# wengroup/matten

Measured on AMD Instinct MI355X. Metric: edge_tensor_products_per_sec, higher is better.
Workload: dtype f32; 1 GPU; configs[2]: synthetic fcc-64 crystals (64 atoms, cutoff 5 A, 1152 edges each), paper hparams lmax=4, eval forward backbone+out_layer, one batch per step per GPU; last conv layer run for its live outputs only (258/842 radial-weight columns: the irreps its only reader takes) -- `value` counts 4 edge-TP per edge all the same, `value_full_layers` is the rate with the full last layer; nodes_per_gpu=64000, edges_per_gpu=1152000, conv_layers=4

## Files before the change

### include/matten_hip.h

```cpp
#ifndef MATTEN_HIP_H
#define MATTEN_HIP_H

#include <stddef.h>
#include <stdint.h>

#ifdef __cplusplus
extern "C" {
#endif

typedef void* matten_stream_t;

#define MATTEN_OK 0
#define MATTEN_EINVAL (-1)
#define MATTEN_ELAUNCH (-2)
#define MATTEN_ENOMEM (-3)

int matten_abi_version(void);

#define MATTEN_RADIAL_MAX_MID 3

size_t matten_csr_workspace_bytes(int64_t n_edges, int64_t n_nodes);
int matten_csr_counting_max_avg_degree(void);
int matten_csr_build(const int64_t* edge_index, int64_t n_edges, int64_t n_nodes, int32_t* perm,
                     int32_t* rowptr, int32_t* src_sorted, void* workspace, size_t workspace_bytes,
// ... 59 lines not shown
                               matten_stream_t stream);
int matten_radial_hidden_deep(const float* geom_sorted, int64_t n_edges, int n_basis, float r_start, float r_end,
                              const float* w0p, int nb_pad, const float* w_mid, int n_mid, int hidden, uint16_t* h2s,
                              const float* h_scale, matten_stream_t stream);
int matten_radial_hidden_multi_deep(const float* geom_sorted, int64_t n_edges, int n_basis, float r_start, float r_end,
                                    const float* const* w0p, int nb_pad, const float* const* w_mid, int n_mid, int hidden,
                                    uint16_t* const* h2s, const float* const* h_scale, int n_layers,
                                    matten_stream_t stream);
int matten_tp_fused(const float* x, int64_t d_in, const uint16_t* h2s, const float* w2p, int64_t w_pad,
                    const float* sh_sorted, int64_t sh_stride, const int32_t* rowptr, const int32_t* src_sorted,
                    int64_t n_nodes, const int32_t* group_entries, const int32_t* unit_map, int64_t n_entries,
                    int64_t units_per_tile, int64_t lds_floats_per_wave, int64_t d_mid, float avg_num_neighbors,
                    const float* num_neigh, const uint16_t* a_split, const float* a_scale_inv,
                    float* agg , matten_stream_t stream);

int matten_tp_max_cols(void);
int matten_tp_max_cols_l0(void);
int matten_tp_max_cols_l1(void);
int matten_tp_groups_hash(void);

int matten_species_linear(const float* x, int64_t d_in, const int32_t* order, const int32_t* seg, int64_t n_species,
                          const float* wp, int64_t w_stride, const int32_t* segs, int64_t n_segs, int64_t d_out,
                          const float* add, int64_t add_ld, int64_t n_rows, float* out, matten_stream_t stream);

int matten_species_linear_rows(const float* x, int64_t d_in, const int32_t* order, const int32_t* seg, int64_t n_species,
                               const float* wp, int64_t w_stride, const int32_t* segs, int64_t n_segs, int64_t d_out,
                               const float* add, int64_t add_ld, int64_t n_rows, float* out, matten_stream_t stream);

int matten_gate_bn(const float* x, int64_t d_in, const int32_t* meta, int64_t d_out, const float* act_cst,
                   const float* running_mean, const float* running_var, const float* bn_weight,
// ... 274 lines not shown
```

### matten_amd/_lib.py

```python
from __future__ import annotations

import ctypes
import os
from ctypes import c_float, c_int, c_int32, c_int64, c_size_t, c_void_p

_HERE = os.path.dirname(os.path.abspath(__file__))
LIB_PATH = os.path.join(_HERE, "libmatten_hip.so")

ABI_VERSION = 47

P = c_void_p
SIGNATURES = {
    "matten_abi_version": (c_int, []),
    "matten_csr_workspace_bytes": (c_size_t, [c_int64, c_int64]),
    "matten_group_workspace_bytes": (c_size_t, [c_int64, c_int64]),
    "matten_csr_counting_max_avg_degree": (c_int, []),
    "matten_csr_build": (c_int, [P, c_int64, c_int64, P, P, P, P, c_size_t, P, P]),
    "matten_csr_split_bound": (c_int64, [c_int64, c_int64, c_int64]),
    "matten_csr_split": (c_int, [P, c_int64, c_int64, c_int64, P, P, P, P, P]),
    "matten_group_by_key": (c_int, [P, c_int64, c_int64, P, P, P, c_size_t, P, P]),
    "matten_species_embed": (c_int, [P, c_int64, P, c_int64, c_int64, c_int64, P, P, c_int64, P, P, P, P, P, P]),
    "matten_edge_geom": (c_int, [P, P, P, P, c_int64, P, P, c_int64, c_int64, c_int, c_int, c_float, c_float, P, P, c_int, P, P, P, P, P]),
    "matten_radial_mlp": (c_int, [P, c_int64, c_int, c_float, c_float, P, c_int, P, P, c_int, c_int, c_float, P, c_int, P]),
    "matten_radial_mlp_deep": (c_int, [P, c_int64, c_int, c_float, c_float, P, c_int, P, c_int, P, c_int, c_int, c_float, P, c_int,
# ... 2 lines not shown
    "matten_tp_paths": (c_int, [P, c_int64, P, c_int64, P, c_int64, P, P, c_int64, P, P, c_int64, c_int64, c_int64, c_float, P, P, c_int,
                                P]),
    "matten_radial_hidden_multi": (c_int, [P, c_int64, c_int, c_float, c_float, P, c_int, P, c_int, P, P, c_int, P]),
    "matten_radial_hidden_multi_deep": (c_int, [P, c_int64, c_int, c_float, c_float, P, c_int, P, c_int, c_int, P, P, c_int, P]),
    "matten_agg_linear_max_mt": (c_int, []),
    "matten_agg_linear_block_chunks": (c_int, []),
    "matten_agg_linear_lds_bytes": (c_size_t, [c_int64, c_int64, c_int64]),
    "matten_agg_linear_max_lds_bytes": (c_size_t, []),
    "matten_agg_linear": (c_int, [P, c_int64, P, P, c_int64, P, c_int64, P, c_int64, P, c_int64, P, c_int64, c_int64,
                                  c_int64, P, P]),
    "matten_agg_linear_gate": (c_int, [P, c_int64, P, P, c_int64, P, c_int64, P, c_int64, P, c_int64, P, c_int64, c_int64,
                                       c_int64, P, P, P, P, c_int64, P, P]),
    "matten_agg_linear_gate_sets": (c_int, []),
    "matten_radial_hidden": (c_int, [P, c_int64, c_int, c_float, c_float, P, c_int, P, c_int, P, P, P]),
    "matten_radial_hidden_deep": (c_int, [P, c_int64, c_int, c_float, c_float, P, c_int, P, c_int, c_int, P, P, P]),
    "matten_tp_max_cols": (c_int, []),
    "matten_tp_max_cols_l0": (c_int, []),
    "matten_tp_max_cols_l1": (c_int, []),
    "matten_tp_groups_hash": (c_int, []),
    "matten_tp_fused": (c_int, [P, c_int64, P, P, c_int64, P, c_int64, P, P, c_int64, P, P, c_int64, c_int64, c_int64, c_int64, c_float, P, P, P, P, P]),
    "matten_species_linear": (c_int, [P, c_int64, P, P, c_int64, P, c_int64, P, c_int64, c_int64, P, c_int64, c_int64, P, P]),
    "matten_species_linear_rows": (c_int, [P, c_int64, P, P, c_int64, P, c_int64, P, c_int64, c_int64, P, c_int64, c_int64, P, P]),
    "matten_radial_mlp_bwd_small_slices": (c_int64, [c_int64]),
    "matten_radial_mlp_bwd_w2_ranges": (c_int64, [c_int64, c_int64]),
    "matten_radial_mlp_bwd_w2_ranges_deep": (c_int64, [c_int64, c_int64, c_int]),
    "matten_radial_mlp_bwd": (c_int, [P, c_int64, c_int, c_float, c_float, P, c_int, P, P, c_int, c_int, c_int, P, c_int64,
                                      c_int, P, P, P, c_float, c_float, c_float, P, P, P]),
    "matten_radial_mlp_bwd_deep": (c_int, [P, c_int64, c_int, c_float, c_float, P, c_int, P, c_int, P, c_int, c_int, c_int, P,
                                           c_int64, c_int, P, P, P, c_float, c_float, c_float, P, P, P]),
    "matten_radial_pack": (c_int, [P, P, P, c_int, c_int, c_int, c_int, c_float, c_float, c_float, P, P, P, P]),
# ... 128 lines not shown
```

### matten_amd/csrc/tp_fused.hip

```cpp
#include "tp_walk.h"

namespace {

using namespace matten_walk;

constexpr int KIND_MERGED = 256;
struct StoreAgg {
    template <class G>
    __device__ __forceinline__ void store(const Args& a, const GroupEntry& ge, const float* __restrict__ acc,
                                          float a_scale_inv, int node, int j, int u, bool valid) const {
        if (TPF_LAB_NO_STORE ? (valid && acc[0] == 12345.678f) : valid) {
            const float nn = a.avg_nn > 0.0f ? a.avg_nn : a.num_neigh[node];
            const float norm = nn > 0.0f ? a_scale_inv / sqrtf(nn) : 0.0f;
            float* orow = a.agg + (int64_t)node * a.d_mid;
            const bool merged = (ge.kind & KIND_MERGED) != 0;
            const GroupEntry& g2 = (&ge)[merged ? 1 : 0];
            const bool second = merged && u >= 2;
            const unsigned mask = merged ? (second ? g2.mask : (unsigned)g2.w_base) : ge.mask;
            const int uc = second ? u - 2 : u;
#pragma unroll
            for (int cc = 0; cc < G::NC; ++cc) {
                if ((mask >> cc) & 1u) {
                    const int d3 = 2 * G::L3[cc] + 1;
                    const int ks = second ? g2.t_off[cc] : ge.t_off[cc];
// ... 22 lines not shown
    const int cu_log2 = ge.cu_log2;
    const int cu = 1 << cu_log2;
    const int npw = 64 >> cu_log2;
    const int ch_log2 = npw >= 16 ? 0 : (4 - (6 - cu_log2));
    const int CH = 1 << ch_log2;
    const int T = npw >= 16 ? (npw >> 4) : 1;
    const int ncols = ge.mul * NC;
    const int MT = (ncols + 15) >> 4;
    const int ycol = MT * 16;
    const int stride = MT * 16 + 32 + 4;

    const int j = lane >> cu_log2;
    const int u = lane & (cu - 1);
    const int g = lane >> 4, c = lane & 15;
    const int xcol = ge.x_off + u * G::D1;
    constexpr int CAPC = cap_channels(L1, NC);
    constexpr int MTMAX = (CAPC * NC + 15) / 16;
    f16x8 ah[MTMAX], al[MTMAX];
    float a_scale_inv;
    {
        float av[MTMAX][8];
        float amax = 0.0f;
#pragma unroll
        for (int mt = 0; mt < MTMAX; ++mt) {
#pragma unroll
            for (int kk = 0; kk < 8; ++kk) {
                const int k = 16 * (kk >> 2) + 4 * g + (kk & 3);
                av[mt][kk] = (mt < MT) ? a.w2p[(int64_t)k * a.w_pad + ge.w_base + mt * 16 + c] : 0.0f;
                amax = fmaxf(amax, fabsf(av[mt][kk]));
            }
// ... 61 lines not shown
        __builtin_amdgcn_s_waitcnt(0xc07f);
        __builtin_amdgcn_wave_barrier();
        for (int so = 0; so < CH; ++so) {
            const int s = s0 + so;
            if (s >= maxdeg) break;
            float x[G::D1];
#pragma unroll
            for (int i = 0; i < G::D1; ++i) x[i] = xn[i];
            {
                const float* xp = a.x + (int64_t)src_nn * a.d_in + xcol;
#pragma unroll
                for (int i = 0; i < G::D1; ++i) xn[i] = xp[i];
                src_nn = a.src_sorted[min(beg + s + 2, e_last)];
            }
            if (s < deg) {
                const float* wp = tile + ((j << ch_log2) + so) * stride + u * NC;
                const float* yp = tile + ((j << ch_log2) + so) * stride + ycol + G::Y0;
                float y[G::NY], w[NC];
#pragma unroll
                for (int jj = 0; jj < G::NY; ++jj) y[jj] = yp[jj];
#pragma unroll
                for (int cc = 0; cc < NC; ++cc) w[cc] = wp[cc];
                G::apply(mask, x, y, w, acc);
            }
        }
        __builtin_amdgcn_wave_barrier();
    }
    StoreAgg{}.store<G>(a, ge, acc, a_scale_inv, node, j, u, valid);
}

#define MATTEN_RGS_ARGS a, ge, tile, stage, (um >> 8) & 0xffff, tile_id, r, reps, lane, StoreAgg{}
#define MATTEN_RGS(L1, GI, TT, TD, P) \
    do { \
        using HM = HotMask<L1, GI>; \
        if (HM::M0 && ge.mask == HM::M0) run_group_shared<L1, GI, TT, TD, P, HM::M0>(MATTEN_RGS_ARGS); \
        else if (HM::M1 && ge.mask == HM::M1) run_group_shared<L1, GI, TT, TD, P, HM::M1>(MATTEN_RGS_ARGS); \
        else run_group_shared<L1, GI, TT, TD, P, 0u>(MATTEN_RGS_ARGS); \
    } while (0)
#if defined(MATTEN_LAB) && defined(TPF_ONLY_VARIANT)
#ifndef TPF_ONLY_MASK
#define TPF_ONLY_MASK 0
#endif
#define MATTEN_RGS_ONLY(L1, GI, TT, TD, P) run_group_shared<L1, GI, TT, TD, P, (unsigned)(TPF_ONLY_MASK)>(MATTEN_RGS_ARGS)
#define MATTEN_GROUP_CASE_SHARED(L1, GI) \
    case (L1 * matten::GROUP_KIND_STRIDE + GI): \
        if (TPF_ONLY_VARIANT == 0) MATTEN_RGS_ONLY(L1, GI, 1, (TPF_CHUNK_DEEP && L1 == 0 ? 2 : 0), true); \
        else if (TPF_ONLY_VARIANT == 1) MATTEN_RGS_ONLY(L1, GI, 2, 0, false); \
        else if (TPF_ONLY_VARIANT == 2) MATTEN_RGS_ONLY(L1, GI, 1, (TPF_CHUNK_DEEP && L1 == 0 ? 2 : TwoDeepOk<L1, GI>::value ? 1 : 0), false); \
        else MATTEN_RGS_ONLY(L1, GI, 1, 0, false); \
        break;
#else
#define MATTEN_GROUP_CASE_SHARED(L1, GI) \
    case (L1 * matten::GROUP_KIND_STRIDE + GI): \
        if (paired && TPF_CHUNK_DEEP && L1 == 0 && nodes_per_wave <= 8 && nodes_per_wave >= 4) MATTEN_RGS(L1, GI, 1, (L1 == 0 ? 2 : 0), true); \
        else if (paired) MATTEN_RGS(L1, GI, 1, 0, true); \
        else if (nodes_per_wave > 16) MATTEN_RGS(L1, GI, 2, 0, false); \
        else if (TPF_CHUNK_DEEP && L1 == 0 && nodes_per_wave <= 8 && nodes_per_wave >= 4) MATTEN_RGS(L1, GI, 1, (L1 == 0 ? 2 : 0), false); \
        else if (TwoDeepOk<L1, GI>::value && nodes_per_wave <= 8 && nodes_per_wave >= TPF_TWO_DEEP_MIN_NPW) MATTEN_RGS(L1, GI, 1, (TwoDeepOk<L1, GI>::value ? 1 : 0), false); \
// ... 401 lines not shown
    if (grid >= ((int64_t)1 << 31)) return MATTEN_EINVAL;
#if TPF_TRACING
    a.trace = nullptr;
    if (g_tp_trace && grid * WAVES_PER_BLOCK <= g_tp_trace_waves) {
        if (g_tp_trace_skip <= 0) a.trace = g_tp_trace;
        if (g_tp_trace_skip == 0) g_tp_trace = nullptr;
        if (g_tp_trace_skip > 0) --g_tp_trace_skip;
    }
#endif
    tp_fused_kernel<<<(unsigned)grid, WAVES_PER_BLOCK * 64, lds, stream>>>(
        a, (const GroupEntry*)group_entries, unit_map, (int)n_entries, (int)units_per_tile, blocks_per_tile, n_tiles);
    MATTEN_LAUNCH_CHECK();
    return MATTEN_OK;
}

extern "C" int matten_tp_max_cols(void) { return TPF_MAX_COLS; }
extern "C" int matten_tp_max_cols_l0(void) { return TPF_MAX_COLS_L0; }
extern "C" int matten_tp_max_cols_l1(void) { return TPF_MAX_COLS_L1; }
extern "C" int matten_tp_groups_hash(void) { return matten::GROUPS_HASH; }
```

### matten_amd/csrc/tp_walk.h

```cpp
#pragma once
#include <type_traits>

#include "cg_gen.h"
#include "common.h"
#include "sh.h"

#ifndef MATTEN_LAB
#if defined(MATTEN_ABLATE_NO_GATHER) || defined(MATTEN_ABLATE_NO_XLOAD) || defined(MATTEN_ABLATE_NO_H2LOAD) || \
    defined(MATTEN_ABLATE_NO_MFMA) || defined(MATTEN_ABLATE_NO_VALU) || defined(MATTEN_ABLATE_NO_STORE) ||      \
    defined(MATTEN_ABLATE_NO_BARRIER) || defined(MATTEN_ABLATE_NO_LOOP) || defined(MATTEN_ABLATE_NO_EPI) || defined(MATTEN_ABLATE_ONE_YQUAD)
#error "MATTEN_ABLATE_* switches are honoured by -DMATTEN_LAB builds only (tools/*.sh)"
#endif
#endif
#if defined(MATTEN_LAB) && defined(MATTEN_ABLATE_NO_GATHER)
#define TPF_SRC(v) ((v) >= 0 ? (node < a.n_nodes ? node : 0) : 0)
#else
#define TPF_SRC(v) (v)
#endif
#if defined(MATTEN_LAB) && defined(MATTEN_ABLATE_NO_XLOAD)
#define TPF_XLD(xp, i, v) (1e-9f * (float)((v) + (i)))
#else
#define TPF_XLD(xp, i, v) ((xp)[i])
#endif
#if defined(MATTEN_LAB) && defined(MATTEN_ABLATE_NO_H2LOAD)
// ... 71 lines not shown

#ifndef TPF_SETPRIO
#define TPF_SETPRIO 3
#endif
#ifndef TPF_W_FIRST
#define TPF_W_FIRST 1
#endif
#ifndef TPF_W_FIRST2
#define TPF_W_FIRST2 1
#endif
#ifndef TPF_PAIR_SUM
#define TPF_PAIR_SUM 1
#endif
#ifndef TPF_EXACT_Y0
#define TPF_EXACT_Y0 0
#endif

#ifndef TPF_REP_PREFETCH
#define TPF_REP_PREFETCH 1
#endif
#ifndef TPF_MAX_COLS
#define TPF_MAX_COLS 64
#endif
#ifndef TPF_MAX_COLS_L0
#define TPF_MAX_COLS_L0 96
#endif
#ifndef TPF_MAX_COLS_L1
#define TPF_MAX_COLS_L1 TPF_MAX_COLS
#endif
__host__ __device__ constexpr int cap_channels(int l1, int nc) {
// ... 71 lines not shown
#pragma unroll
    for (int off = 32; off > 0; off >>= 1) maxdeg = max(maxdeg, __shfl_xor(maxdeg, off));
    if constexpr (TPF_LAB_NO_LOOP) maxdeg = 0;
    n.maxdeg = maxdeg;
    return n;
}
__device__ __forceinline__ UnitNodes unit_nodes(const Args& a, const GroupEntry& ge, int tile_id, int r, int lane) {
    return unit_nodes_finish(unit_nodes_issue(a, ge, tile_id, r, lane));
}

constexpr int STAGE_ROW = 68;
constexpr int STAGE_TMAX = 2;
constexpr int STAGE_FLOATS = 16 * STAGE_TMAX * STAGE_ROW;
constexpr int STAGE_TOTAL_FLOATS = 2 * STAGE_FLOATS;

template <int MTC>
__device__ __forceinline__ void mfma_tiles(const f16x8* __restrict__ ah, const f16x8* __restrict__ al, f16x8 bh, f16x8 bl,
                                           float* __restrict__ trow) {
    const f32x4 zero = {0.f, 0.f, 0.f, 0.f};
    f32x4 dx[MTC], dh[MTC];
#pragma unroll
    for (int mt = 0; mt < MTC; ++mt) {
        dx[mt] = __builtin_amdgcn_mfma_f32_16x16x32_f16(al[mt], bh, zero, 0, 0, 0);
        dh[mt] = __builtin_amdgcn_mfma_f32_16x16x32_f16(ah[mt], bh, zero, 0, 0, 0);
    }
#pragma unroll
    for (int mt = 0; mt < MTC; ++mt) dx[mt] = __builtin_amdgcn_mfma_f32_16x16x32_f16(ah[mt], bl, dx[mt], 0, 0, 0);
#pragma unroll
    for (int mt = 0; mt < MTC; ++mt) *reinterpret_cast<f32x4*>(trow + mt * 16) = dh[mt] + SPLIT_LO_INV * dx[mt];
}
// ... 6 lines not shown
    const char* safe;
    int64_t row_bytes;
    float* st_w;
    int beg_ld[TT], deg_ld[TT], so_ld[TT];
    int CH;
    f32x4 pf[TT];

    __device__ __forceinline__ void init(const Args& a, float* stage, int cu_log2, int beg, int deg_node) {
        const int npw = 64 >> cu_log2;
        const int ch_log2 = npw >= 16 ? 0 : 4 - (6 - cu_log2);
        CH = 1 << ch_log2;
        const int piece = threadIdx.x & 15;
        base = piece < 8 ? reinterpret_cast<const char*>(a.h2s) + piece * 16
                         : reinterpret_cast<const char*>(a.sh) + (piece - 8) * 16;
        row_bytes = piece < 8 ? (int64_t)(2 * HID * sizeof(_Float16)) : (int64_t)a.sh_stride * 4;
        safe = reinterpret_cast<const char*>(a.w2p);
        st_w = stage + (threadIdx.x >> 4) * STAGE_ROW + piece * 4;
#pragma unroll
        for (int t = 0; t < TT; ++t) {
            const int n = (int)(threadIdx.x >> 4) + 16 * t;
            const int jn = (n >> ch_log2) & (npw - 1);
            so_ld[t] = n & (CH - 1);
            beg_ld[t] = __shfl(beg, jn << cu_log2);
            deg_ld[t] = __shfl(deg_node, jn << cu_log2);
            pf[t] = f32x4{0.f, 0.f, 0.f, 0.f};
        }
    }
    __device__ __forceinline__ void issue(int s0) {
        if constexpr (TPF_LAB_NO_H2LOAD) return;
#pragma unroll
        for (int t = 0; t < TT; ++t)
// ... 22 lines not shown
        const int npw = 64 >> cu_log2;
        const int ch_log2 = 4 - (6 - cu_log2);
        CH = 1 << ch_log2;
        const int wave = threadIdx.x >> 6, lane = threadIdx.x & 63;
        if ((wave & 1) == 0 && (lane & ((1 << cu_log2) - 1)) == 0) {
            info[((wave >> 1) * 16 + (lane >> cu_log2)) * 2] = beg;
            info[((wave >> 1) * 16 + (lane >> cu_log2)) * 2 + 1] = deg_node;
            if (lane == 0) info[2 * 16 * 2 + (wave >> 1)] = my_maxdeg;
        }
        __syncthreads();
        maxdeg = max(info[2 * 16 * 2], info[2 * 16 * 2 + 1]);
        const int piece = threadIdx.x & 15;
        base = piece < 8 ? reinterpret_cast<const char*>(a.h2s) + piece * 16
                         : reinterpret_cast<const char*>(a.sh) + (piece - 8) * 16;
        row_bytes = piece < 8 ? (int64_t)(2 * HID * sizeof(_Float16)) : (int64_t)a.sh_stride * 4;
        safe = reinterpret_cast<const char*>(a.w2p);
        const int n = (int)(threadIdx.x >> 4);
        st_w = stage + n * STAGE_ROW + piece * 4;
        const int jn = (n >> ch_log2) & (npw - 1);
        so_ld = n & (CH - 1);
#pragma unroll
        for (int t = 0; t < 2; ++t) {
            beg_ld[t] = info[(t * 16 + jn) * 2];
            deg_ld[t] = info[(t * 16 + jn) * 2 + 1];
            pf[t] = f32x4{0.f, 0.f, 0.f, 0.f};
        }
    }
    __device__ __forceinline__ void issue(int s0) {
#pragma unroll
        for (int t = 0; t < 2; ++t)
            pf[t] = *reinterpret_cast<const f32x4*>(
// ... 36 lines not shown
        __syncthreads();
        int buf = 0;
        for (int s0 = 0; s0 < un.maxdeg; s0 += ld.CH, buf ^= 1) {
            ld.issue(s0 + ld.CH);
            ld.publish(buf ^ 1);
            __syncthreads();
        }
    }
}
__device__ __forceinline__ void run_loader_only(const Args& a, const GroupEntry& ge, float* __restrict__ stage, int tile_id,
                                                int r0, int reps, int lane) {
    if ((64 >> ge.cu_log2) > 16) run_loader_only_t<2>(a, ge, stage, tile_id, r0, reps, lane);
    else run_loader_only_t<1>(a, ge, stage, tile_id, r0, reps, lane);
}

template <int L1, int GI>
struct TwoDeepOk { static constexpr bool value = L1 == 0 || (L1 == 1 && (GI == 0 || TPF_PAIR_SUM)); };

template <int L1, int GI, int TT, int TWO_DEEP, bool PAIRED, unsigned CMASK, class Epilogue>
__device__ __forceinline__ void run_group_shared(const Args& a, const GroupEntry& ge, float* __restrict__ tile,
                                                 float* __restrict__ stage, int entry, int tile_id, int r0, int reps, int lane,
                                                 const Epilogue& epi) {
    static_assert(!PAIRED || TT == 1, "paired workgroups stage 2 x 16 rows");
#if TPF_TRACING
    const unsigned tr_in_hi = tpf_stamp_hi();
    const unsigned tr_in = tpf_stamp();
    unsigned tr_mfma = 0, tr_con = 0, tr_pub = 0, tr_bar = 0, tr_chunks = 0, tr_pro = 0, tr_epi = 0;
    unsigned tr_pro_pre = 0, tr_epi_sg = 0;
#endif
    const int row0 = PAIRED ? 16 * (int)(threadIdx.x >> 7) : 0;
    constexpr int STAGE_BUF = (PAIRED ? 32 : 16 * TT) * STAGE_ROW;
    using G = matten::Group<L1, GI>;
    constexpr int NC = G::NC;

    const unsigned mask = ge.mask;
    const int cu_log2 = ge.cu_log2;
    const int cu = 1 << cu_log2;
    const int npw = 64 >> cu_log2;
    const int ch_log2 = npw >= 16 ? 0 : 4 - (6 - cu_log2);
    const int CH = 1 << ch_log2;
    const int ncols = ge.mul * NC;
#if defined(MATTEN_LAB) && defined(TPF_ONLY_MT)
    const int MT = TPF_ONLY_MT;
#else
    const int MT = (ncols + 15) >> 4;
#endif

    const int j = lane >> cu_log2;
    const int u = lane & (cu - 1);
    const int g = lane >> 4, c = lane & 15;
    const int xcol = ge.x_off + u * G::D1;
    constexpr int CAPC = cap_channels(L1, NC);
    constexpr int MTMAX = (CAPC * NC + 15) / 16;
    const int stride = MT * 16 + 4;
    f16x8 ah[MTMAX], al[MTMAX];
    float a_scale_inv;
    if (a.a_split) {
        const f16x8* ap = reinterpret_cast<const f16x8*>(a.a_split) + ((int64_t)ge.a_tile * 64 + lane) * 2;
#pragma unroll
        for (int mt = 0; mt < MTMAX; ++mt) {
            const f16x8 z = {0, 0, 0, 0, 0, 0, 0, 0};
            ah[mt] = mt < MT ? ap[mt * 128] : z;
            al[mt] = mt < MT ? ap[mt * 128 + 1] : z;
        }
        a_scale_inv = a.a_scale_inv[entry];
    } else
    {
        float av[MTMAX][8];
        float amax = 0.0f;
// ... 12 lines not shown
        e = amax > 0.0f ? max(-100, min(100, e)) : 13;
        const float a_scale = __uint_as_float((unsigned)(127 + 13 - e) << 23);
        a_scale_inv = __uint_as_float((unsigned)(127 - 13 + e) << 23);
#pragma unroll
        for (int mt = 0; mt < MTMAX; ++mt) {
#pragma unroll
            for (int kk = 0; kk < 8; ++kk) {
                _Float16 hi, lo;
                split_f16(av[mt][kk] * a_scale, hi, lo);
                ah[mt][kk] = hi;
                al[mt][kk] = lo;
            }
        }
    }

    typename std::conditional<PAIRED, PairLoader, StageLoader<TT>>::type ld;
    static_assert(!TWO_DEEP || TwoDeepOk<L1, GI>::value, "two rows in flight only for the light kinds");
    static_assert(TWO_DEEP != 2 || G::D1 == 1, "a chunk of rows in flight: scalar input blocks");
    constexpr bool two_deep = TWO_DEEP == 1;
    constexpr bool chunk_deep = TWO_DEEP == 2;
    constexpr int XQ = 4;
    float xqa[XQ], xqb[XQ];
    int sq[XQ];
    int node, beg, deg, maxdeg, e_last;
    bool valid;
    float xn[G::D1], xb[G::D1];
    int src_nn, src_b = 0;
    auto start_group = [&](const UnitNodes& un) {
        node = un.node, beg = un.beg, valid = un.valid, maxdeg = un.maxdeg;
        deg = valid ? un.deg : 0;
// ... 51 lines not shown
#if TPF_TRACING
    const unsigned tr_loop = tpf_stamp();
    unsigned tr_a = tr_loop;
    tr_pro += (unsigned)(tr_loop - tr_rep);
#endif
    auto chunk_body = [&](const int s0, const int buf, float (&xcur)[XQ], float (&xnext)[XQ]) {
        __builtin_amdgcn_s_setprio(TPF_SETPRIO);
        ld.issue(s0 + CH);
        const float* sb = stage + buf * STAGE_BUF + row0 * STAGE_ROW;
#pragma unroll
        for (int t = 0; t < TT; ++t) {
            {
                const f16x8 bh = *reinterpret_cast<const f16x8*>(sb + (16 * t + c) * STAGE_ROW + g * 4);
                const f16x8 bl = *reinterpret_cast<const f16x8*>(sb + (16 * t + c) * STAGE_ROW + 16 + g * 4);
                if constexpr (TPF_LAB_NO_MFMA) {
                    if ((float)bh[0] == 12345.f) tile[c] = (float)bl[0];
                    continue;
                }
                float* trow = tile + (16 * t + c) * stride + 4 * g;
                if (MTMAX == 1 || MT == 1) mfma_tiles<1>(ah, al, bh, bl, trow);
                else if (MTMAX == 2 || MT == 2) mfma_tiles<(MTMAX < 2 ? MTMAX : 2)>(ah, al, bh, bl, trow);
                else if (MTMAX == 3 || MT == 3) mfma_tiles<(MTMAX < 3 ? MTMAX : 3)>(ah, al, bh, bl, trow);
                else if (MTMAX == 4 || MT == 4) mfma_tiles<(MTMAX < 4 ? MTMAX : 4)>(ah, al, bh, bl, trow);
                else if (MTMAX == 5 || MT == 5) mfma_tiles<(MTMAX < 5 ? MTMAX : 5)>(ah, al, bh, bl, trow);
                else if (MTMAX == 6 || MT == 6) mfma_tiles<(MTMAX < 6 ? MTMAX : 6)>(ah, al, bh, bl, trow);
                else mfma_tiles<MTMAX>(ah, al, bh, bl, trow);
            }
        }
        __builtin_amdgcn_s_waitcnt(0xc07f);
        __builtin_amdgcn_wave_barrier();
        __builtin_amdgcn_s_setprio(0);
#if TPF_TRACING
        const unsigned tr_b = tpf_stamp();
#endif
        auto contract = [&](int so, const float* __restrict__ x) {
            const float* wp = tile + ((j << ch_log2) + so) * stride + u * NC;
            const float* yp = sb + ((j << ch_log2) + so) * STAGE_ROW + 32 + G::Y0;
            float y[G::NY], w[NC];
            if constexpr (TPF_W_FIRST) {
#pragma unroll
                for (int cc = 0; cc < NC; ++cc) w[cc] = wp[cc];
                asm volatile("" ::: "memory");
            }
            if constexpr (TPF_EXACT_Y0 && L1 == 0 && G::Y0 == 0 && G::NY % 4 == 1) {
                y[G::NY - 1] = yp[G::NY - 1];
#pragma unroll
                for (int q = 0; q < G::NY / 4; ++q) {
                    const f32x4 v = reinterpret_cast<const f32x4*>(yp)[q];
                    y[4 * q] = v[0], y[4 * q + 1] = v[1], y[4 * q + 2] = v[2], y[4 * q + 3] = v[3];
                }
            } else
            {
                constexpr int Q0 = G::Y0 / 4 * 4, NQ = (G::Y0 + G::NY - Q0 + 3) / 4;
                float yq[4 * NQ];
                const f32x4* y4 = reinterpret_cast<const f32x4*>(yp - (G::Y0 - Q0));
#pragma unroll
                for (int q = 0; q < NQ; ++q) {
#if defined(MATTEN_LAB) && defined(MATTEN_ABLATE_ONE_YQUAD)
                    const f32x4 v0 = y4[0];
                    const f32x4 v = q == 0 ? v0 : v0 * (float)(q + 1);
#else
                    const f32x4 v = y4[q];
#endif
                    yq[4 * q] = v[0], yq[4 * q + 1] = v[1], yq[4 * q + 2] = v[2], yq[4 * q + 3] = v[3];
                }
#pragma unroll
                for (int jj = 0; jj < G::NY; ++jj) y[jj] = yq[G::Y0 - Q0 + jj];
            }
            if constexpr (!TPF_W_FIRST) {
#pragma unroll
                for (int cc = 0; cc < NC; ++cc) w[cc] = wp[cc];
            }
            G::apply(CMASK ? CMASK : mask, x, y, w, acc);
        };
        if constexpr (TPF_LAB_NO_VALU) {
        } else if constexpr (TWO_DEEP && TPF_PAIR_SUM && G::HAS_APPLY2) {
            auto fetch = [&](int so, float (&y)[G::NY], float (&w)[NC]) {
                const float* wp = tile + ((j << ch_log2) + so) * stride + u * NC;
                const float* yp = sb + ((j << ch_log2) + so) * STAGE_ROW + 32 + G::Y0;
                if constexpr (TPF_W_FIRST2) {
#pragma unroll
                    for (int cc = 0; cc < NC; ++cc) w[cc] = wp[cc];
                    asm volatile("" ::: "memory");
                }
                constexpr int Q0 = G::Y0 / 4 * 4, NQ = (G::Y0 + G::NY - Q0 + 3) / 4;
                float yq[4 * NQ];
                const f32x4* y4 = reinterpret_cast<const f32x4*>(yp - (G::Y0 - Q0));
#pragma unroll
                for (int q = 0; q < NQ; ++q) {
                    const f32x4 v = y4[q];
                    yq[4 * q] = v[0], yq[4 * q + 1] = v[1], yq[4 * q + 2] = v[2], yq[4 * q + 3] = v[3];
                }
#pragma unroll
                for (int jj = 0; jj < G::NY; ++jj) y[jj] = yq[G::Y0 - Q0 + jj];
                if constexpr (!TPF_W_FIRST2) {
#pragma unroll
                    for (int cc = 0; cc < NC; ++cc) w[cc] = wp[cc];
                }
            };
            for (int so = 0; so < CH; so += 2) {
                const int s = s0 + so;
                float ya[G::NY], wa[NC], yb[G::NY], wb[NC], xa[G::D1], xc[G::D1];
                fetch(so, ya, wa);
                fetch(so + 1, yb, wb);
#pragma unroll
                for (int i = 0; i < G::D1; ++i) xa[i] = s < deg ? xn[i] : 0.0f, xc[i] = s + 1 < deg ? xb[i] : 0.0f;
                {
                    const float* xp = a.x + (int64_t)TPF_SRC(src_nn) * a.d_in + xcol;
#pragma unroll
                    for (int i = 0; i < G::D1; ++i) xn[i] = TPF_XLD(xp, i, src_nn);
                    src_nn = a.src_sorted[min(beg + s + 4, e_last)];
                }
                {
                    const float* xp = a.x + (int64_t)TPF_SRC(src_b) * a.d_in + xcol;
#pragma unroll
                    for (int i = 0; i < G::D1; ++i) xb[i] = TPF_XLD(xp, i, src_b);
                    src_b = a.src_sorted[min(beg + s + 5, e_last)];
                }
                G::apply2(CMASK ? CMASK : mask, xa, ya, wa, xc, yb, wb, acc);
            }
        } else if constexpr (chunk_deep) {
#pragma unroll
            for (int i = 0; i < XQ; ++i) {
                const float* xp = a.x + (int64_t)TPF_SRC(sq[i]) * a.d_in + xcol;
                xnext[i] = TPF_XLD(xp, 0, sq[i]);
            }
#pragma unroll
            for (int i = 0; i < XQ; ++i) sq[i] = a.src_sorted[min(beg + s0 + 2 * CH + i, e_last)];
#pragma unroll
            for (int so = 0; so < XQ; ++so) {
                if (so < CH && s0 + so < deg) contract(so, xcur + so);
            }
        } else if (two_deep) {
            for (int so = 0; so < CH; so += 2) {
                const int s = s0 + so;
                if (s < deg) contract(so, xn);
                {
                    const float* xp = a.x + (int64_t)TPF_SRC(src_nn) * a.d_in + xcol;
#pragma unroll
                    for (int i = 0; i < G::D1; ++i) xn[i] = TPF_XLD(xp, i, src_nn);
                    src_nn = a.src_sorted[min(beg + s + 4, e_last)];
                }
                if (s + 1 < deg) contract(so + 1, xb);
                {
                    const float* xp = a.x + (int64_t)TPF_SRC(src_b) * a.d_in + xcol;
#pragma unroll
                    for (int i = 0; i < G::D1; ++i) xb[i] = TPF_XLD(xp, i, src_b);
                    src_b = a.src_sorted[min(beg + s + 5, e_last)];
                }
            }
        } else {
            for (int so = 0; so < CH; ++so) {
                const int s = s0 + so;
                if (s >= maxdeg) break;
                float x[G::D1];
#pragma unroll
                for (int i = 0; i < G::D1; ++i) x[i] = xn[i];
                {
                    const float* xp = a.x + (int64_t)TPF_SRC(src_nn) * a.d_in + xcol;
#pragma unroll
                    for (int i = 0; i < G::D1; ++i) xn[i] = TPF_XLD(xp, i, src_nn);
                    src_nn = a.src_sorted[min(beg + s + 2, e_last)];
                }
                if (s < deg) contract(so, x);
            }
// ... 94 lines not shown
```

### matten_amd/ops.py

```python
from __future__ import annotations

from typing import Optional, Tuple

import os

import numpy as np

import torch

from . import _lib
from .nn._tables import bump_weights_epoch


_EVENTS = None
_EVENTS_ONLY = None


def enable_event_timing(flag: bool = True, only=None) -> None:
    global _EVENTS, _EVENTS_ONLY
    _EVENTS = {} if flag else None
    _EVENTS_ONLY = tuple(only) if (flag and only) else None


def event_timings_ms():
# ... 540 lines not shown
_GROUPS_CHECKED = False


def tp_fused(x, h2p, w2p, sh_sorted, rowptr, src_sorted, entries, unit_map, units_per_tile: int,
             lds_floats_per_wave: int, d_mid: int, avg_num_neighbors: float, num_neigh=None,
             a_split=None) -> torch.Tensor:
    lib = _lib.load()
    from .plan import TP_TILE_NODES

    if lib.matten_tp_tile_nodes() != TP_TILE_NODES:
        raise _lib.MattenHipError("plan.TP_TILE_NODES does not match the library's node tile")
    from .plan import TP_MAX_COLS, TP_MAX_COLS_L0, TP_MAX_COLS_L1
    if (lib.matten_tp_max_cols() != TP_MAX_COLS or lib.matten_tp_max_cols_l0() != TP_MAX_COLS_L0
            or lib.matten_tp_max_cols_l1() != TP_MAX_COLS_L1):
        raise _lib.MattenHipError("plan.TP_MAX_COLS does not match the library's entry width (-DTPF_MAX_COLS)")
    global _GROUPS_CHECKED
    from .plan import tp_groups_hash
    if not _GROUPS_CHECKED and lib.matten_tp_groups_hash() != tp_groups_hash():
        raise _lib.MattenHipError("the library's coupling code (cg_gen.h) was generated for other coupling groups than plan.TP_GROUPS "
                                  "(MATTEN_TP_GROUPS / an interrupted tools/*.sh A/B build?): make -C matten_amd/csrc clean all")
    _GROUPS_CHECKED = True
    x = _need_rows(x, torch.float32, "node_features")
    h2p = _need(h2p, torch.float16, "h2s")
    if h2p.dim() != 3 or h2p.shape[1:] != (2, 32):
        raise ValueError(f"h2s must be [E,2,32] fp16 (ops.split_hidden / ops.radial_hidden), got {tuple(h2p.shape)}")
    w2p = _need(w2p, torch.float32, "w2p")
    sh_sorted = _need(sh_sorted, torch.float32, "sh_sorted")
    N, d_in = rowptr.shape[0] - 1, x.stride(0)
    if num_neigh is not None:
        num_neigh = _need(num_neigh, torch.float32, "num_neigh")
# ... 1071 lines not shown
```

### matten_amd/plan.py

```python
from __future__ import annotations

import math
import os
from dataclasses import dataclass, field
from typing import Dict, List, Optional, Sequence, Tuple

import numpy as np

from .o3 import Irrep, Irreps, wigner_3j

TP_TILE_NODES = 64

def _range_groups(ranges, l1, lmax=4):
    return [[(l2, l3) for l2 in range(lo, hi + 1) for l3 in range(abs(l1 - l2), min(lmax, l1 + l2) + 1)] for lo, hi in ranges]


def _moved(l1, to_first, lmax=4):
    g0, g1 = _range_groups([(0, 2), (3, 4)], l1, lmax)
    assert all(c in g1 for c in to_first)
    return [g0 + list(to_first), [c for c in g1 if c not in to_first]]


_GROUP_SCHEMES = {
    "A": {l1: _range_groups([(0, 4)] if l1 == 0 else [(0, 2), (3, 4)], l1) for l1 in range(5)},
# ... 41 lines not shown
            return [(gi, TP_GROUPS[l1][gi])]
    return list(enumerate(TP_GROUPS[l1][:n_reg]))
TP_MAX_COMBOS = 12
TP_MAX_COLS = int(os.environ.get("MATTEN_TP_MAX_COLS", "64"))
TP_MAX_COLS_L0 = int(os.environ.get("MATTEN_TP_MAX_COLS_L0", "96"))
TP_MAX_COLS_L1 = int(os.environ.get("MATTEN_TP_MAX_COLS_L1", str(TP_MAX_COLS)))
TP_KIND_STRIDE = 8

ACT_CODE = {None: 0, "silu": 1, "tanh": 2, "sigmoid": 3, "ssp": 4, "abs": 5}


LIGHT_LMAX = 1

TP_KIND_MERGED = 256
TP_MERGE = os.environ.get("MATTEN_TP_MERGE", "1") != "0"

FUSED_UNIT_SHARED = 1 << 24
FUSED_UNIT_LOADER_ONLY = 1 << 25
FUSED_UNIT_PAIRED = 1 << 26
FUSED_UNIT_REPS_SHIFT = 27


def fused_persist(cu_log2: int, groups: int, mode: str) -> int:
    spec = os.environ.get("MATTEN_TP_PERSIST", TP_PERSIST_DEFAULT)
    want = 1
    for item in filter(None, spec.split(",")):
        lanes, reps = item.split(":")
        if int(lanes) == (1 << cu_log2):
            want = int(reps)
    avail = groups // 2 if mode == "paired" else groups
# ... 277 lines not shown
            la = by_block[a_][0].l1
            own = lambda blk: groups_for_block(la, [(p.l2, p.l3) for p in by_block[blk]])
            if all(len(own(blk)) == 1 and own(blk)[0][0] >= TP_GROUPS_REGULAR[la] for blk in (a_, b_)):
                del partner[a_]
    second = set(partner.values())

    def add_entry(l1, gi, combos, x_off, u0, mul_c, cu_log2, halves):
        nonlocal fused_a_tiles, lds_need
        d1_ = 2 * l1 + 1
        nodes_per_wave = max(1, 64 // (1 << cu_log2))
        n_tiles16 = max(1, nodes_per_wave // 16)
        live = list(combos)
        lds_need = max(lds_need, 16 * n_tiles16 * (16 * (-(-(mul_c * len(live)) // 16)) + 32 + 4))
        n_mt = -(-(mul_c * len(live)) // 16)
        merged = len(halves) == 2
        rows = []
        for h, (mul_h, present) in enumerate(halves):
            row = [-1, 0, mul_h, cu_log2, 0, 0, 0, 0] + [0] * 24
            mask = 0
            for c, key in enumerate(combos):
                if key in present:
                    pth = present[key]
                    mask |= 1 << c
                    row[8 + 12 + c] = pth.out_off + u0 * (2 * pth.l3 + 1)
            row[4] = mask
            rows.append(row)
        head = rows[0]
        head[0] = l1 * TP_KIND_STRIDE + gi + (TP_KIND_MERGED if merged else 0)
        head[1], head[2], head[5], head[6], head[7] = x_off + u0 * d1_, mul_c, len(fused_cols), fused_a_tiles, n_mt
        if merged:
            rows[1][5] = head[4]
            head[4] |= rows[1][4]
        fused_a_tiles += n_mt
        for (mul_h, present) in halves:
            for uu in range(mul_h):
                for key in live:
                    fused_cols.append(present[key].w_off + u0 + uu if key in present else -1)
        for r_, (mul_h, present) in zip(rows, halves):
            gentries.append(r_)
            gentry_paths.append({c: paths.index(present[key]) for c, key in enumerate(combos) if key in present})
            gentry_u0.append(u0)
            gentry_mul.append(mul_h)
        gstart.append(gstart[-1] + -(-TP_TILE_NODES // nodes_per_wave))

    for i_in1 in block_ids:
        if i_in1 in second:
            continue
        plist = by_block[i_in1]
        l1, mul = plist[0].l1, plist[0].mul
        both = list(plist) + (list(by_block[partner[i_in1]]) if i_in1 in partner else [])
        for gi, combos in groups_for_block(l1, [(p.l2, p.l3) for p in both]):
            present = {(p.l2, p.l3): p for p in plist if (p.l2, p.l3) in combos}
# ... 514 lines not shown
```

Measured before the change: 1.246 billion edge-TP/s.

## Hand radial weights from MFMA accumulators straight to registers for light kinds

For unmerged entries with l1<=1 and 8 or 16 lanes per node whose channel count equals the lane count, the plan now orders the weight columns coupling-major. The fused TP kernel then keeps the MFMA results in registers (using DPP row-rotation for the 8-lane case) instead of writing them to the LDS tile and reading them back. This drops the LDS round-trip and the wave barrier/waitcnt for those entries. The cost is more template variants and register pressure, with the low half of A optionally spilled to LDS for wide entries. A library-build check rejects plans that mark such entries when the kernel was built without support.

```diff
diff --git a/include/matten_hip.h b/include/matten_hip.h
--- a/include/matten_hip.h
+++ b/include/matten_hip.h
@@ -97,6 +97,7 @@
                     const float* num_neigh, const uint16_t* a_split, const float* a_scale_inv,
                     float* agg , matten_stream_t stream);
 
+int matten_tp_wreg(void);
 int matten_tp_max_cols(void);
 int matten_tp_max_cols_l0(void);
 int matten_tp_max_cols_l1(void);
diff --git a/matten_amd/_lib.py b/matten_amd/_lib.py
--- a/matten_amd/_lib.py
+++ b/matten_amd/_lib.py
@@ -40,6 +40,7 @@
     "matten_agg_linear_gate_sets": (c_int, []),
     "matten_radial_hidden": (c_int, [P, c_int64, c_int, c_float, c_float, P, c_int, P, c_int, P, P, P]),
     "matten_radial_hidden_deep": (c_int, [P, c_int64, c_int, c_float, c_float, P, c_int, P, c_int, c_int, P, P, P]),
+    "matten_tp_wreg": (c_int, []),
     "matten_tp_max_cols": (c_int, []),
     "matten_tp_max_cols_l0": (c_int, []),
     "matten_tp_max_cols_l1": (c_int, []),
diff --git a/matten_amd/csrc/tp_fused.hip b/matten_amd/csrc/tp_fused.hip
--- a/matten_amd/csrc/tp_fused.hip
+++ b/matten_amd/csrc/tp_fused.hip
@@ -5,6 +5,7 @@
 using namespace matten_walk;
 
 constexpr int KIND_MERGED = 256;
+constexpr int KIND_WREG = 512;
 struct StoreAgg {
     template <class G>
     __device__ __forceinline__ void store(const Args& a, const GroupEntry& ge, const float* __restrict__ acc,
@@ -60,6 +61,8 @@
     const int u = lane & (cu - 1);
     const int g = lane >> 4, c = lane & 15;
     const int xcol = ge.x_off + u * G::D1;
+    const bool cmajor = WregOk<L1, GI, 3>::value && (ge.kind & KIND_WREG) != 0;
+    const int wcol0 = cmajor ? u : u * NC, wstep = cmajor ? cu : 1;
     constexpr int CAPC = cap_channels(L1, NC);
     constexpr int MTMAX = (CAPC * NC + 15) / 16;
     f16x8 ah[MTMAX], al[MTMAX];
@@ -151,13 +154,13 @@
                 src_nn = a.src_sorted[min(beg + s + 2, e_last)];
             }
             if (s < deg) {
-                const float* wp = tile + ((j << ch_log2) + so) * stride + u * NC;
+                const float* wp = tile + ((j << ch_log2) + so) * stride + wcol0;
                 const float* yp = tile + ((j << ch_log2) + so) * stride + ycol + G::Y0;
                 float y[G::NY], w[NC];
 #pragma unroll
                 for (int jj = 0; jj < G::NY; ++jj) y[jj] = yp[jj];
 #pragma unroll
-                for (int cc = 0; cc < NC; ++cc) w[cc] = wp[cc];
+                for (int cc = 0; cc < NC; ++cc) w[cc] = wp[cc * wstep];
                 G::apply(mask, x, y, w, acc);
             }
         }
@@ -167,18 +170,40 @@
 }
 
 #define MATTEN_RGS_ARGS a, ge, tile, stage, (um >> 8) & 0xffff, tile_id, r, reps, lane, StoreAgg{}
-#define MATTEN_RGS(L1, GI, TT, TD, P) \
+#define MATTEN_RGS_WR(L1, GI, TT, TD, P, WR) \
     do { \
         using HM = HotMask<L1, GI>; \
-        if (HM::M0 && ge.mask == HM::M0) run_group_shared<L1, GI, TT, TD, P, HM::M0>(MATTEN_RGS_ARGS); \
-        else if (HM::M1 && ge.mask == HM::M1) run_group_shared<L1, GI, TT, TD, P, HM::M1>(MATTEN_RGS_ARGS); \
-        else run_group_shared<L1, GI, TT, TD, P, 0u>(MATTEN_RGS_ARGS); \
+        if (HM::M0 && ge.mask == HM::M0) run_group_shared<L1, GI, TT, TD, P, HM::M0, WR>(MATTEN_RGS_ARGS); \
+        else if (HM::M1 && ge.mask == HM::M1) run_group_shared<L1, GI, TT, TD, P, HM::M1, WR>(MATTEN_RGS_ARGS); \
+        else run_group_shared<L1, GI, TT, TD, P, 0u, WR>(MATTEN_RGS_ARGS); \
     } while (0)
+template <int L1, int GI, int TT, int TD, bool P>
+__device__ __forceinline__ void run_group_shared_any(const Args& a, const GroupEntry& ge, float* __restrict__ tile,
+                                                     float* __restrict__ stage, int um, int tile_id, int r, int reps, int lane) {
+    if constexpr (TT == 1 && WregOk<L1, GI, 4>::value) {
+        if ((ge.kind & KIND_WREG) && ge.cu_log2 == 4) {
+            MATTEN_RGS_WR(L1, GI, TT, TD, P, 4);
+            return;
+        }
+    }
+    if constexpr (TT == 1 && WregOk<L1, GI, 3>::value) {
+        if ((ge.kind & KIND_WREG) && ge.cu_log2 == 3) {
+            MATTEN_RGS_WR(L1, GI, TT, TD, P, 3);
+            return;
+        }
+    }
+    if (ge.kind & KIND_WREG) return;
+    MATTEN_RGS_WR(L1, GI, TT, TD, P, 0);
+}
+#define MATTEN_RGS(L1, GI, TT, TD, P) run_group_shared_any<L1, GI, TT, TD, P>(a, ge, tile, stage, um, tile_id, r, reps, lane)
 #if defined(MATTEN_LAB) && defined(TPF_ONLY_VARIANT)
 #ifndef TPF_ONLY_MASK
 #define TPF_ONLY_MASK 0
 #endif
-#define MATTEN_RGS_ONLY(L1, GI, TT, TD, P) run_group_shared<L1, GI, TT, TD, P, (unsigned)(TPF_ONLY_MASK)>(MATTEN_RGS_ARGS)
+#ifndef TPF_ONLY_WR
+#define TPF_ONLY_WR 0
+#endif
+#define MATTEN_RGS_ONLY(L1, GI, TT, TD, P) run_group_shared<L1, GI, TT, TD, P, (unsigned)(TPF_ONLY_MASK), (TT == 1 ? TPF_ONLY_WR : 0)>(MATTEN_RGS_ARGS)
 #define MATTEN_GROUP_CASE_SHARED(L1, GI) \
     case (L1 * matten::GROUP_KIND_STRIDE + GI): \
         if (TPF_ONLY_VARIANT == 0) MATTEN_RGS_ONLY(L1, GI, 1, (TPF_CHUNK_DEEP && L1 == 0 ? 2 : 0), true); \
@@ -610,6 +635,7 @@
     return MATTEN_OK;
 }
 
+extern "C" int matten_tp_wreg(void) { return TPF_WREG ? TPF_WREG_MAX_L1 + 1 : 0; }
 extern "C" int matten_tp_max_cols(void) { return TPF_MAX_COLS; }
 extern "C" int matten_tp_max_cols_l0(void) { return TPF_MAX_COLS_L0; }
 extern "C" int matten_tp_max_cols_l1(void) { return TPF_MAX_COLS_L1; }
diff --git a/matten_amd/csrc/tp_walk.h b/matten_amd/csrc/tp_walk.h
--- a/matten_amd/csrc/tp_walk.h
+++ b/matten_amd/csrc/tp_walk.h
@@ -109,6 +109,16 @@
 #endif
 #ifndef TPF_EXACT_Y0
 #define TPF_EXACT_Y0 0
+#endif
+
+#ifndef TPF_WREG
+#define TPF_WREG 1
+#endif
+#ifndef TPF_WREG_ALO_LDS_MT
+#define TPF_WREG_ALO_LDS_MT 5
+#endif
+#ifndef TPF_WREG_MAX_L1
+#define TPF_WREG_MAX_L1 1
 #endif
 
 #ifndef TPF_REP_PREFETCH
@@ -210,6 +220,10 @@
 constexpr int STAGE_FLOATS = 16 * STAGE_TMAX * STAGE_ROW;
 constexpr int STAGE_TOTAL_FLOATS = 2 * STAGE_FLOATS;
 
+__device__ __forceinline__ const char* stage_safe_row(const Args& a) {
+    return reinterpret_cast<const char*>(a.w2p + ((max(a.w_pad, 4) - 4) & ~3));
+}
+
 template <int MTC>
 __device__ __forceinline__ void mfma_tiles(const f16x8* __restrict__ ah, const f16x8* __restrict__ al, f16x8 bh, f16x8 bl,
                                            float* __restrict__ trow) {
@@ -246,7 +260,7 @@
         base = piece < 8 ? reinterpret_cast<const char*>(a.h2s) + piece * 16
                          : reinterpret_cast<const char*>(a.sh) + (piece - 8) * 16;
         row_bytes = piece < 8 ? (int64_t)(2 * HID * sizeof(_Float16)) : (int64_t)a.sh_stride * 4;
-        safe = reinterpret_cast<const char*>(a.w2p);
+        safe = stage_safe_row(a);
         st_w = stage + (threadIdx.x >> 4) * STAGE_ROW + piece * 4;
 #pragma unroll
         for (int t = 0; t < TT; ++t) {
@@ -299,7 +313,7 @@
         base = piece < 8 ? reinterpret_cast<const char*>(a.h2s) + piece * 16
                          : reinterpret_cast<const char*>(a.sh) + (piece - 8) * 16;
         row_bytes = piece < 8 ? (int64_t)(2 * HID * sizeof(_Float16)) : (int64_t)a.sh_stride * 4;
-        safe = reinterpret_cast<const char*>(a.w2p);
+        safe = stage_safe_row(a);
         const int n = (int)(threadIdx.x >> 4);
         st_w = stage + n * STAGE_ROW + piece * 4;
         const int jn = (n >> ch_log2) & (npw - 1);
@@ -366,14 +380,31 @@
     else run_loader_only_t<1>(a, ge, stage, tile_id, r0, reps, lane);
 }
 
+template <int SO> using Slot = std::integral_constant<int, SO>;
+__device__ __forceinline__ int slot_next(int so) { return so + 1; }
+template <int SO> __device__ __forceinline__ Slot<SO + 1> slot_next(Slot<SO>) { return {}; }
+template <int I, int N, int STEP, class F>
+__device__ __forceinline__ void for_slots(F&& f) {
+    if constexpr (I < N) {
+        f(Slot<I>{});
+        for_slots<I + STEP, N, STEP>(f);
+    }
+}
+template <int L1, int GI, int WR>
+struct WregOk {
+    static constexpr bool value = TPF_WREG && L1 <= TPF_WREG_MAX_L1 && (WR == 3 || WR == 4) &&
+                                  cap_channels(L1, matten::Group<L1, GI>::NC) >= (1 << WR);
+};
+
 template <int L1, int GI>
 struct TwoDeepOk { static constexpr bool value = L1 == 0 || (L1 == 1 && (GI == 0 || TPF_PAIR_SUM)); };
 
-template <int L1, int GI, int TT, int TWO_DEEP, bool PAIRED, unsigned CMASK, class Epilogue>
+template <int L1, int GI, int TT, int TWO_DEEP, bool PAIRED, unsigned CMASK, int WR, class Epilogue>
 __device__ __forceinline__ void run_group_shared(const Args& a, const GroupEntry& ge, float* __restrict__ tile,
                                                  float* __restrict__ stage, int entry, int tile_id, int r0, int reps, int lane,
                                                  const Epilogue& epi) {
     static_assert(!PAIRED || TT == 1, "paired workgroups stage 2 x 16 rows");
+    static_assert(WR == 0 || (TT == 1 && (WR == 3 || WR == 4)), "register hand-over: one MFMA tile per chunk, 8 or 16 lanes per node");
 #if TPF_TRACING
     const unsigned tr_in_hi = tpf_stamp_hi();
     const unsigned tr_in = tpf_stamp();
@@ -386,16 +417,18 @@
     constexpr int NC = G::NC;
 
     const unsigned mask = ge.mask;
-    const int cu_log2 = ge.cu_log2;
+    const int cu_log2 = WR ? WR : ge.cu_log2;
     const int cu = 1 << cu_log2;
     const int npw = 64 >> cu_log2;
     const int ch_log2 = npw >= 16 ? 0 : 4 - (6 - cu_log2);
     const int CH = 1 << ch_log2;
     const int ncols = ge.mul * NC;
+    constexpr int WCH = WR == 4 ? 4 : WR == 3 ? 2 : 1;
+    constexpr int MTW = WR == 4 ? NC : WR == 3 ? (NC + 1) / 2 : 0;
 #if defined(MATTEN_LAB) && defined(TPF_ONLY_MT)
     const int MT = TPF_ONLY_MT;
 #else
-    const int MT = (ncols + 15) >> 4;
+    const int MT = WR ? MTW : (ncols + 15) >> 4;
 #endif
 
     const int j = lane >> cu_log2;
@@ -404,7 +437,11 @@
     const int xcol = ge.x_off + u * G::D1;
     constexpr int CAPC = cap_channels(L1, NC);
     constexpr int MTMAX = (CAPC * NC + 15) / 16;
+    static_assert(MTW <= MTMAX, "a register hand-over entry is no wider than the plan's cap");
     const int stride = MT * 16 + 4;
+    float wr[WR ? NC * WCH : 1];
+    constexpr bool ALO_LDS = WR != 0 && MTW >= TPF_WREG_ALO_LDS_MT;
+    f16x8* const alo_lds = reinterpret_cast<f16x8*>(tile) + lane;
     f16x8 ah[MTMAX], al[MTMAX];
     float a_scale_inv;
     if (a.a_split) {
@@ -447,6 +484,10 @@
         }
     }
 
+    if constexpr (ALO_LDS) {
+#pragma unroll
+        for (int mt = 0; mt < MTW; ++mt) alo_lds[mt * 64] = al[mt];
+    }
     typename std::conditional<PAIRED, PairLoader, StageLoader<TT>>::type ld;
     static_assert(!TWO_DEEP || TwoDeepOk<L1, GI>::value, "two rows in flight only for the light kinds");
     static_assert(TWO_DEEP != 2 || G::D1 == 1, "a chunk of rows in flight: scalar input blocks");
@@ -528,7 +569,41 @@
                 const f16x8 bh = *reinterpret_cast<const f16x8*>(sb + (16 * t + c) * STAGE_ROW + g * 4);
                 const f16x8 bl = *reinterpret_cast<const f16x8*>(sb + (16 * t + c) * STAGE_ROW + 16 + g * 4);
                 if constexpr (TPF_LAB_NO_MFMA) {
-                    if ((float)bh[0] == 12345.f) tile[c] = (float)bl[0];
+                    if constexpr (WR) {
+#pragma unroll
+                        for (int k = 0; k < NC * WCH; ++k) wr[k] = (float)bh[0] + (float)bl[0];
+                    } else if ((float)bh[0] == 12345.f) tile[c] = (float)bl[0];
+                    continue;
+                }
+                if constexpr (WR) {
+                    const f32x4 zero = {0.f, 0.f, 0.f, 0.f};
+                    f32x4 dx[MTW], dh[MTW];
+#pragma unroll
+                    for (int mt = 0; mt < MTW; ++mt) {
+                        const f16x8 alo = ALO_LDS ? alo_lds[mt * 64] : al[mt];
+                        dx[mt] = __builtin_amdgcn_mfma_f32_16x16x32_f16(bh, alo, zero, 0, 0, 0);
+                        dh[mt] = __builtin_amdgcn_mfma_f32_16x16x32_f16(bh, ah[mt], zero, 0, 0, 0);
+                    }
+#pragma unroll
+                    for (int mt = 0; mt < MTW; ++mt) dx[mt] = __builtin_amdgcn_mfma_f32_16x16x32_f16(bl, ah[mt], dx[mt], 0, 0, 0);
+#pragma unroll
+                    for (int mt = 0; mt < MTW; ++mt) {
+                        const f32x4 d = dh[mt] + SPLIT_LO_INV * dx[mt];
+                        if constexpr (WR == 4) {
+#pragma unroll
+                            for (int i = 0; i < 4; ++i) wr[mt * WCH + i] = d[i];
+                        } else {
+                            constexpr int ROR8 = 0x128;
+#pragma unroll
+                            for (int so = 0; so < 2; ++so) {
+                                wr[2 * mt * WCH + so] = __int_as_float(__builtin_amdgcn_update_dpp(
+                                    __float_as_int(d[so]), __float_as_int(d[2 + so]), ROR8, 0xf, 0xc, false));
+                                if (2 * mt + 1 < NC)
+                                    wr[(2 * mt + 1) * WCH + so] = __int_as_float(__builtin_amdgcn_update_dpp(
+                                        __float_as_int(d[2 + so]), __float_as_int(d[so]), ROR8, 0xf, 0x3, false));
+                            }
+                        }
+                    }
                     continue;
                 }
                 float* trow = tile + (16 * t + c) * stride + 4 * g;
@@ -541,17 +616,26 @@
                 else mfma_tiles<MTMAX>(ah, al, bh, bl, trow);
             }
         }
-        __builtin_amdgcn_s_waitcnt(0xc07f);
-        __builtin_amdgcn_wave_barrier();
+        if constexpr (WR == 0) {
+            __builtin_amdgcn_s_waitcnt(0xc07f);
+            __builtin_amdgcn_wave_barrier();
+        }
         __builtin_amdgcn_s_setprio(0);
 #if TPF_TRACING
-        const unsigned tr_b = tpf_stamp();
-#endif
-        auto contract = [&](int so, const float* __restrict__ x) {
+        unsigned tr_b;
+        if constexpr (WR) tr_b = tpf_stamp_after(wr);
+        else tr_b = tpf_stamp();
+#endif
+        auto contract = [&](auto so_c, const float* __restrict__ x) {
+            const int so = so_c;
             const float* wp = tile + ((j << ch_log2) + so) * stride + u * NC;
             const float* yp = sb + ((j << ch_log2) + so) * STAGE_ROW + 32 + G::Y0;
             float y[G::NY], w[NC];
-            if constexpr (TPF_W_FIRST) {
+            if constexpr (WR) {
+#pragma unroll
+                for (int cc = 0; cc < NC; ++cc) w[cc] = wr[cc * WCH + decltype(so_c)::value];
+                asm volatile("" ::: "memory");
+            } else if constexpr (TPF_W_FIRST) {
 #pragma unroll
                 for (int cc = 0; cc < NC; ++cc) w[cc] = wp[cc];
                 asm volatile("" ::: "memory");
@@ -581,7 +665,7 @@
 #pragma unroll
                 for (int jj = 0; jj < G::NY; ++jj) y[jj] = yq[G::Y0 - Q0 + jj];
             }
-            if constexpr (!TPF_W_FIRST) {
+            if constexpr (!WR && !TPF_W_FIRST) {
 #pragma unroll
                 for (int cc = 0; cc < NC; ++cc) w[cc] = wp[cc];
             }
@@ -589,10 +673,14 @@
         };
         if constexpr (TPF_LAB_NO_VALU) {
         } else if constexpr (TWO_DEEP && TPF_PAIR_SUM && G::HAS_APPLY2) {
-            auto fetch = [&](int so, float (&y)[G::NY], float (&w)[NC]) {
+            auto fetch = [&](auto so_c, float (&y)[G::NY], float (&w)[NC]) {
+                const int so = so_c;
                 const float* wp = tile + ((j << ch_log2) + so) * stride + u * NC;
                 const float* yp = sb + ((j << ch_log2) + so) * STAGE_ROW + 32 + G::Y0;
-                if constexpr (TPF_W_FIRST2) {
+                if constexpr (WR) {
+#pragma unroll
+                    for (int cc = 0; cc < NC; ++cc) w[cc] = wr[cc * WCH + decltype(so_c)::value];
+                } else if constexpr (TPF_W_FIRST2) {
 #pragma unroll
                     for (int cc = 0; cc < NC; ++cc) w[cc] = wp[cc];
                     asm volatile("" ::: "memory");
@@ -607,16 +695,17 @@
                 }
 #pragma unroll
                 for (int jj = 0; jj < G::NY; ++jj) y[jj] = yq[G::Y0 - Q0 + jj];
-                if constexpr (!TPF_W_FIRST2) {
+                if constexpr (!WR && !TPF_W_FIRST2) {
 #pragma unroll
                     for (int cc = 0; cc < NC; ++cc) w[cc] = wp[cc];
                 }
             };
-            for (int so = 0; so < CH; so += 2) {
+            auto pair_pass = [&](auto so_c) {
+                const int so = so_c;
                 const int s = s0 + so;
                 float ya[G::NY], wa[NC], yb[G::NY], wb[NC], xa[G::D1], xc[G::D1];
-                fetch(so, ya, wa);
-                fetch(so + 1, yb, wb);
+                fetch(so_c, ya, wa);
+                fetch(slot_next(so_c), yb, wb);
 #pragma unroll
                 for (int i = 0; i < G::D1; ++i) xa[i] = s < deg ? xn[i] : 0.0f, xc[i] = s + 1 < deg ? xb[i] : 0.0f;
                 {
@@ -632,7 +721,9 @@
                     src_b = a.src_sorted[min(beg + s + 5, e_last)];
                 }
                 G::apply2(CMASK ? CMASK : mask, xa, ya, wa, xc, yb, wb, acc);
-            }
+            };
+            if constexpr (WR) for_slots<0, WCH, 2>(pair_pass);
+            else for (int so = 0; so < CH; so += 2) pair_pass(so);
         } else if constexpr (chunk_deep) {
 #pragma unroll
             for (int i = 0; i < XQ; ++i) {
@@ -641,28 +732,54 @@
             }
 #pragma unroll
             for (int i = 0; i < XQ; ++i) sq[i] = a.src_sorted[min(beg + s0 + 2 * CH + i, e_last)];
-#pragma unroll
-            for (int so = 0; so < XQ; ++so) {
-                if (so < CH && s0 + so < deg) contract(so, xcur + so);
+            if constexpr (WR) {
+                for_slots<0, WCH, 1>([&](auto so_c) {
+                    if (s0 + so_c < deg) contract(so_c, xcur + so_c);
+                });
+            } else {
+#pragma unroll
+                for (int so = 0; so < XQ; ++so) {
+                    if (so < CH && s0 + so < deg) contract(so, xcur + so);
+                }
             }
         } else if (two_deep) {
-            for (int so = 0; so < CH; so += 2) {
+            auto pair_steps = [&](auto so_c) {
+                const int so = so_c;
                 const int s = s0 + so;
-                if (s < deg) contract(so, xn);
+                if (s < deg) contract(so_c, xn);
                 {
                     const float* xp = a.x + (int64_t)TPF_SRC(src_nn) * a.d_in + xcol;
 #pragma unroll
                     for (int i = 0; i < G::D1; ++i) xn[i] = TPF_XLD(xp, i, src_nn);
                     src_nn = a.src_sorted[min(beg + s + 4, e_last)];
                 }
-                if (s + 1 < deg) contract(so + 1, xb);
+                if (s + 1 < deg) contract(slot_next(so_c), xb);
                 {
                     const float* xp = a.x + (int64_t)TPF_SRC(src_b) * a.d_in + xcol;
 #pragma unroll
                     for (int i = 0; i < G::D1; ++i) xb[i] = TPF_XLD(xp, i, src_b);
                     src_b = a.src_sorted[min(beg + s + 5, e_last)];
                 }
-            }
+            };
+            if constexpr (WR) for_slots<0, WCH, 2>(pair_steps);
+            else for (int so = 0; so < CH; so += 2) pair_steps(so);
+        } else if constexpr (WR != 0) {
+            bool go = true;
+            for_slots<0, WCH, 1>([&](auto so_c) {
+                const int s = s0 + so_c;
+                go = go && s < maxdeg;
+                if (!go) return;
+                float x[G::D1];
+#pragma unroll
+                for (int i = 0; i < G::D1; ++i) x[i] = xn[i];
+                {
+                    const float* xp = a.x + (int64_t)TPF_SRC(src_nn) * a.d_in + xcol;
+#pragma unroll
+                    for (int i = 0; i < G::D1; ++i) xn[i] = TPF_XLD(xp, i, src_nn);
+                    src_nn = a.src_sorted[min(beg + s + 2, e_last)];
+                }
+                if (s < deg) contract(so_c, x);
+            });
         } else {
             for (int so = 0; so < CH; ++so) {
                 const int s = s0 + so;
diff --git a/matten_amd/ops.py b/matten_amd/ops.py
--- a/matten_amd/ops.py
+++ b/matten_amd/ops.py
@@ -578,6 +578,10 @@
     if (lib.matten_tp_max_cols() != TP_MAX_COLS or lib.matten_tp_max_cols_l0() != TP_MAX_COLS_L0
             or lib.matten_tp_max_cols_l1() != TP_MAX_COLS_L1):
         raise _lib.MattenHipError("plan.TP_MAX_COLS does not match the library's entry width (-DTPF_MAX_COLS)")
+    from .plan import TP_WREG_MAX_L1, tp_wreg
+    if tp_wreg() and lib.matten_tp_wreg() != TP_WREG_MAX_L1 + 1:
+        raise _lib.MattenHipError("plans mark coupling-major entries (plan.TP_KIND_WREG) that this library was not built for "
+                                  "(-DTPF_WREG=0 / -DTPF_WREG_MAX_L1): set MATTEN_TP_WREG=0")
     global _GROUPS_CHECKED
     from .plan import tp_groups_hash
     if not _GROUPS_CHECKED and lib.matten_tp_groups_hash() != tp_groups_hash():
diff --git a/matten_amd/plan.py b/matten_amd/plan.py
--- a/matten_amd/plan.py
+++ b/matten_amd/plan.py
@@ -79,6 +79,13 @@
 
 TP_KIND_MERGED = 256
 TP_MERGE = os.environ.get("MATTEN_TP_MERGE", "1") != "0"
+TP_KIND_WREG = 512
+TP_WREG_MAX_L1 = 1
+TP_WREG_DEFAULT = "1"
+
+
+def tp_wreg() -> bool:
+    return os.environ.get("MATTEN_TP_WREG", TP_WREG_DEFAULT) != "0"
 
 FUSED_UNIT_SHARED = 1 << 24
 FUSED_UNIT_LOADER_ONLY = 1 << 25
@@ -386,6 +393,7 @@
         lds_need = max(lds_need, 16 * n_tiles16 * (16 * (-(-(mul_c * len(live)) // 16)) + 32 + 4))
         n_mt = -(-(mul_c * len(live)) // 16)
         merged = len(halves) == 2
+        wreg = (tp_wreg() and not merged and l1 <= TP_WREG_MAX_L1 and cu_log2 in (3, 4) and mul_c == (1 << cu_log2))
         rows = []
         for h, (mul_h, present) in enumerate(halves):
             row = [-1, 0, mul_h, cu_log2, 0, 0, 0, 0] + [0] * 24
@@ -398,16 +406,17 @@
             row[4] = mask
             rows.append(row)
         head = rows[0]
-        head[0] = l1 * TP_KIND_STRIDE + gi + (TP_KIND_MERGED if merged else 0)
+        head[0] = l1 * TP_KIND_STRIDE + gi + (TP_KIND_MERGED if merged else 0) + (TP_KIND_WREG if wreg else 0)
         head[1], head[2], head[5], head[6], head[7] = x_off + u0 * d1_, mul_c, len(fused_cols), fused_a_tiles, n_mt
         if merged:
             rows[1][5] = head[4]
             head[4] |= rows[1][4]
         fused_a_tiles += n_mt
         for (mul_h, present) in halves:
-            for uu in range(mul_h):
-                for key in live:
-                    fused_cols.append(present[key].w_off + u0 + uu if key in present else -1)
+            order = ([(uu, key) for key in live for uu in range(mul_h)] if wreg else
+                     [(uu, key) for uu in range(mul_h) for key in live])
+            for uu, key in order:
+                fused_cols.append(present[key].w_off + u0 + uu if key in present else -1)
         for r_, (mul_h, present) in zip(rows, halves):
             gentries.append(r_)
             gentry_paths.append({c: paths.index(present[key]) for c, key in enumerate(combos) if key in present})
```

Result: faster. 1.275 billion edge-TP/s, median of 6 (+2.3%).
